# antoine311200/sow

Measured on AMD Instinct MI355X. Metric: SoWLinear fwd+bwd tokens/s, llama_60m rank=50 (56-layer SoWLinear stack), higher is better.
Workload: dtype bf16

## Files before the change

sow_amd/csrc/api.hip:

```cpp
#include "kernels.hpp"
#include <cstring>
#include <vector>
#include <cstdio>
#include <cstdlib>

namespace sow {

template <typename T, typename TO>
__global__ __launch_bounds__(256) void colsum_kernel(const T* M, int64_t ld, int64_t rows, int D, TO* out, float beta) {
  __shared__ float red[4][64];
  const int c = blockIdx.x * 64 + (threadIdx.x & 63), w = threadIdx.x >> 6;
  float s = 0.f;
  if (c < D)
    for (int64_t i = w; i < rows; i += 4) s += to_f32(M[i * ld + c]);
  red[w][threadIdx.x & 63] = s;
  __syncthreads();
  if (w == 0 && c < D) {
    float v = red[0][threadIdx.x] + red[1][threadIdx.x] + red[2][threadIdx.x] + red[3][threadIdx.x];
    if (beta != 0.f) v += beta * to_f32(out[c]);
    out[c] = from_f32<TO>(v);
  }
}
static int launch_colsum(const void* dy, int64_t T, int d_out, void* dbias, float beta, int dtype, int out_dtype,
                         hipStream_t stream) {
  const dim3 grid((d_out + 63) / 64);
  if (out_dtype != dtype && out_dtype != SOW_F32) return SOW_ERR_DTYPE;
  const bool o32 = out_dtype == SOW_F32;
  if (dtype == SOW_F32)
    hipLaunchKernelGGL((colsum_kernel<float, float>), grid, dim3(256), 0, stream, (const float*)dy, (int64_t)d_out, T, d_out, (float*)dbias, beta);
  else if (dtype == SOW_BF16 && o32)
    hipLaunchKernelGGL((colsum_kernel<bf16_t, float>), grid, dim3(256), 0, stream, (const bf16_t*)dy, (int64_t)d_out, T, d_out, (float*)dbias, beta);
  else if (dtype == SOW_BF16)
    hipLaunchKernelGGL((colsum_kernel<bf16_t, bf16_t>), grid, dim3(256), 0, stream, (const bf16_t*)dy, (int64_t)d_out, T, d_out, (bf16_t*)dbias, beta);
  else if (dtype == SOW_F16 && o32)
    hipLaunchKernelGGL((colsum_kernel<f16_t, float>), grid, dim3(256), 0, stream, (const f16_t*)dy, (int64_t)d_out, T, d_out, (float*)dbias, beta);
  else if (dtype == SOW_F16)
    hipLaunchKernelGGL((colsum_kernel<f16_t, f16_t>), grid, dim3(256), 0, stream, (const f16_t*)dy, (int64_t)d_out, T, d_out, (f16_t*)dbias, beta);
  else
    return SOW_ERR_DTYPE;
  SOW_CHECK_LAUNCH();
  return SOW_OK;
}
}

namespace sow {
static const char* const kSwitchNames[SW_COUNT] = {"FORCE_CHAIN_V1", "NO_SHORT_SPLIT", "NO_FUSED_H", "FORCE_GEMM_V1", "TN_NARROW",
                                                   "NO_GEMM3S",      "GEMM3S",         "GEMM3",      "NO_GROUPED",     "NO_PERSIST",     "NO_NT_STORE",    "NT_LOAD",        "NO_PAIR_FLUSH",  "F32_EXACT",
                                                   "NO_PARK16",      "TN_NO_NT_LOAD",  "NO_TN_ROWS",     "GEMM4",          "NO_GEMM4H",      "NO_CHAIN3F",     "NO_TN_F32Q",     "NO_SPLITK",
                                                   "NO_WIDE_CHAIN",  "NO_SHARED_X",    "NO_RAGGED",      "NO_RAGGED_GEMM", "NO_BLOCKED_QR",
                                                   "NO_SKINNY",      "NO_FUSED_ACC",   "NO_F16_TN",
                                                   "NO_H_ROWS"};
static std::atomic<int> g_switch[SW_COUNT];
static std::once_flag g_switch_once;
static void switches_from_env() {
  for (int i = 0; i < SW_COUNT; ++i) {
    char name[64];
    snprintf(name, sizeof name, "SOW_AMD_%s", kSwitchNames[i]);
    const char* v = getenv(name);
    const bool tri = i == SW_GEMM3S || i == SW_GEMM3 || i == SW_GEMM4;
    g_switch[i].store(!v ? -1 : (tri ? (v[0] != '0') : 1), std::memory_order_relaxed);
  }
}
int sw(int which) {
  std::call_once(g_switch_once, switches_from_env);
  return g_switch[which].load(std::memory_order_relaxed);
}
}

using namespace sow;

static inline size_t al256(size_t v) { return (v + 255) & ~(size_t)255; }
static inline size_t esize(int dtype) { return dtype == SOW_F32 ? 4 : 2; }
static inline bool ok_dtype(int d) { return d == SOW_F32 || d == SOW_BF16 || d == SOW_F16; }
static inline bool al4p(const void* p) { return (reinterpret_cast<uintptr_t>(p) & 3) == 0; }
static inline bool al16p(const void* p) { return (reinterpret_cast<uintptr_t>(p) & 15) == 0; }
static inline int split_dtype(int d, bool* pf) {
  d &= ~SOW_FUSE_ACC;
  *pf = (d & SOW_PARAM_F32) != 0;
  const int cd = d & ~SOW_PARAM_F32;
  if (!ok_dtype(cd) || (*pf && cd == SOW_F32)) return -1;
  return cd;
}
static inline bool flagged(int d) { return (d & SOW_PARAM_F32) != 0; }
static inline bool fuse_of(int d) { return (d & SOW_FUSE_ACC) != 0 && !flagged(d); }
static inline int nofuse(int d) { return d & ~SOW_FUSE_ACC; }

constexpr int SHORT_NTB = 128;
static inline int short_want(int ntb) { return ntb > 0 ? (256 + ntb - 1) / ntb : 1; }
static size_t short_hp_bytes(int64_t T, int d_in, int d_out, int r_live, int dtype) {
  const int ntb = ceil_div(T, 64);
  if (r_live > 64 || ntb <= 0 || ntb > SHORT_NTB) return 0;
  const int dmax = d_in > d_out ? d_in : d_out;
  int ks = short_want(ntb);
// ... 29 lines not shown
  if (nsl == 0) return SOW_OK;
  ChainParams b = p;
  const int kn = want < nsl ? want : nsl;
  b.ntb = ntb, b.st_per = 0, b.sl_per = ceil_div(nsl, kn), b.Hpartial = nullptr, b.Hload = p.Hsave, b.Hsave = nullptr;
  return f32 ? launch_chain2f(b, bwd, stream) : launch_chain2(b, bwd, dtype, stream);
}

static int gemm_auto(const void* A, int64_t lda, const void* B, int64_t ldb, bool transB, void* C, int64_t ldc,
                     const void* bias, int64_t M, int N, int K, float alpha, float beta, int dtype, hipStream_t stream,
                     void* ws = nullptr, size_t ws_bytes = 0) {
  if (dtype == SOW_F16) {
    const int g4 = sw(SW_GEMM4);
    const int64_t work = (int64_t)ceil_div(M, 256) * ceil_div(N, 256) * gemm4_splits(M, N, K, false, ws, ws_bytes);
    if (!sw_on(SW_FORCE_GEMM_V1) && (g4 > 0 || (g4 < 0 && work >= 120)) &&
        gemm4_supported(A, lda, B, ldb, transB, nullptr, 0, nullptr, 0, C, ldc, bias, M, N, K, dtype))
      return launch_gemm4(A, lda, B, ldb, transB, nullptr, 0, nullptr, 0, 0, C, ldc, bias, M, N, K, alpha, beta, stream, ws,
                          ws_bytes, dtype);
    return launch_gemm(A, lda, false, B, ldb, transB, C, ldc, bias, M, N, K, alpha, beta, dtype, stream);
  }
  if (gemm2_supported(A, lda, B, ldb, transB, nullptr, 0, nullptr, 0, C, ldc, bias, M, N, K, dtype))
    return launch_gemm2(A, lda, B, ldb, transB, nullptr, 0, nullptr, 0, 0, C, ldc, bias, M, N, K, alpha, beta, stream, ws, ws_bytes);
  return launch_gemm(A, lda, false, B, ldb, transB, C, ldc, bias, M, N, K, alpha, beta, dtype, stream);
}

extern "C" {

int sow_version(void) { return 120; }

int sow_set_switch(const char* name, int value) {
  if (!name) return SOW_ERR_NULL;
  (void)sw(0);
  for (int i = 0; i < SW_COUNT; ++i)
    if (!strcmp(name, kSwitchNames[i])) {
      g_switch[i].store(value < 0 ? -1 : (value != 0), std::memory_order_relaxed);
      return SOW_OK;
    }
  return SOW_ERR_UNSUPPORTED;
}

#ifdef SOW_STAMPS
int sow_debug_set_stamps(void* buf) {
  g_chain2_stamps = buf;
  return SOW_OK;
}
#endif

int sow_get_switch(const char* name) {
  if (!name) return SOW_ERR_NULL;
  for (int i = 0; i < SW_COUNT; ++i)
    if (!strcmp(name, kSwitchNames[i])) return sw(i);
  return SOW_ERR_UNSUPPORTED;
}

const char* sow_error_string(int code) {
  switch (code) {
    case SOW_OK: return "ok";
    case SOW_ERR_NULL: return "null pointer argument";
    case SOW_ERR_SHAPE: return "invalid shape argument";
    case SOW_ERR_DTYPE: return "unsupported dtype";
    case SOW_ERR_ALIGN: return "misaligned pointer";
    case SOW_ERR_WORKSPACE: return "workspace too small";
    case SOW_ERR_UNSUPPORTED: return "unsupported configuration";
    default: return code > 0 ? hipGetErrorString((hipError_t)code) : "unknown error";
  }
}

size_t sow_h_save_elems(int64_t T, int r_live) { return (size_t)T * (size_t)(r_live <= 64 ? 64 : r_live); }
// ... 1233 lines not shown
```

sow_amd/csrc/chain2.hip:

```cpp
#include "kernels.hpp"
#include "lds_dma.hpp"

namespace sow {

#ifdef SOW_STAMPS
#define C2_STAMP(i)                                                                                  \
  do {                                                                                               \
    if (stamps && w == 0 && lane == 0) stamps[i] = __builtin_amdgcn_s_memrealtime();                \
  } while (0)
#else
#define C2_STAMP(i) \
  do {              \
  } while (0)
#endif
#ifdef SOW_STAMPS
#define C2_TICK() __builtin_amdgcn_s_memrealtime()
#define C2_ACC(var, t0) var += __builtin_amdgcn_s_memrealtime() - (t0)
#define C2_PUT(cond, i, var)                     \
  do {                                           \
    if (stamps && (cond) && lane == 0) stamps[i] = (var); \
  } while (0)
#else
#define C2_TICK() 0ull
#define C2_ACC(var, t0) (void)(t0)
// ... 4 lines not shown

constexpr int C2_NTG = 2;
constexpr int C2_NCW = 2 * C2_NTG;
constexpr int C2_NLW = 2;
constexpr int C2_BM = 32 * C2_NTG;
#ifndef C2_DEPTH_X
#define C2_DEPTH_X 4
#define C2_NSLOT_X 6
#define C2_AHEAD_X 5
#endif
constexpr int C2_DEPTH = C2_DEPTH_X;
constexpr int C2_STAGE = 4096;
constexpr int C2_NSLOT = C2_NSLOT_X;
constexpr int C2_AHEAD = C2_AHEAD_X;
#ifdef C2_EXPERIMENT_SHALLOW_X
static_assert(C2_NSLOT == C2_AHEAD + 1 && C2_NSLOT + C2_DEPTH == 10 && C2_DEPTH >= 3 && C2_DEPTH <= 6, "80 KiB");
#else
static_assert(C2_NSLOT == C2_AHEAD + 1 && C2_NSLOT + C2_DEPTH == 10 && C2_DEPTH >= 4 && C2_DEPTH <= 6,
              "80 KiB: 8 KiB per chunk slot + 2 x 4 KiB per X slot; two 8-KiB fp32 park tiles per token group must fit its X ring");
#endif
constexpr int C2_FSLOT = 8192;
constexpr int C2_LPW = 8 / C2_NLW;
constexpr int C2_RING0 = C2_NSLOT * C2_FSLOT;
constexpr int C2_RING = C2_DEPTH * C2_STAGE;
constexpr int C2_LDS = C2_RING0 + C2_NTG * C2_RING;
constexpr int C2_THREADS = 64 * (C2_NCW + C2_NLW);
constexpr int C2_RESIDENT = 512;


template <bool TR> __device__ __forceinline__ int img_chunk(int row, int c) {
  return TR ? (c ^ (((row >> 1) & 1) << 2)) : (c ^ ((row >> 1) & 7));
}

template <typename T, bool BWD, bool P16>
__device__ __forceinline__ void chain2_block(const ChainParams& p, const int bid, char* smem, const int t, const int lane, const int w,
                                             uint64_t* stamps) {
  constexpr bool TR = !BWD;
  C2_STAMP(0);
  const int tb = p.ntb > 0 ? bid % p.ntb : bid;
  const int split = p.ntb > 0 ? bid / p.ntb : 0;
  const int64_t m0 = (int64_t)tb * C2_BM;
  const int D1 = p.D1, D2 = p.D2, rb = p.rb;
  const int nst_all = (D1 + 63) / 64, nsl_all = (D2 + 63) / 64;
  const int st0 = p.st_per > 0 ? split * p.st_per : 0;
  const int sl0 = p.sl_per > 0 ? split * p.sl_per : 0;
  const int nst = p.sl_per > 0 ? 0 : (p.st_per > 0 ? (nst_all - st0 < p.st_per ? nst_all - st0 : p.st_per) : nst_all);
  const int nsl = p.st_per > 0 ? 0 : (p.sl_per > 0 ? (nsl_all - sl0 < p.sl_per ? nsl_all - sl0 : p.sl_per) : nsl_all);
  const int total = nst + nsl;
  const T* Amat = (const T*)(BWD ? p.F2b : p.F1b);
  const T* Bmat = (const T*)(BWD ? p.F1b : p.F2b);
  const int64_t ldb = BWD ? p.ldf1b : p.ldf2b;
  const int rows_a = BWD ? D2 : D1, cols_b = BWD ? D1 : D2;
  const char* zp = zero_page_for(lane);

  if (w >= C2_NCW) {
    __builtin_amdgcn_s_setprio(3);
    const int lw = w - C2_NCW;
    const char* a_end = (const char*)(Amat + (int64_t)rows_a * rb);
    const bool own_last = rows_a > 0 && lw == ((rows_a - 1) & 63) / (8 * C2_LPW);
    uint32_t last_row_dw = 0u;
    if (own_last && lane < 32 && 2 * lane < rb) last_row_dw = *((const uint32_t*)(Amat + (int64_t)(rows_a - 1) * rb) + lane);
    asm volatile("" : "+v"(last_row_dw));
    auto chunk_is_a = [&](int c) { return BWD ? (c >= nst) : (c < nst); };
    const char* a_ptr[C2_LPW];
    const char* b_ptr[C2_LPW];
    int b_stride[C2_LPW], b_lc[C2_LPW];
#pragma unroll
    for (int ii = 0; ii < C2_LPW; ++ii) {
      const int i = C2_LPW * lw + ii;
      const int row = 8 * i + (lane >> 3), pc = lane & 7;
      const int lc = img_chunk<TR>(row, pc);
      a_ptr[ii] = (const char*)(Amat + (int64_t)row * rb) + 16 * lc;
      const bool bv = row < rb;
      b_ptr[ii] = bv ? (const char*)(Bmat + (int64_t)row * ldb + 8 * lc) : zp;
      b_stride[ii] = bv ? 128 : 0;
      b_lc[ii] = lc;
    }
    const int a_chunk_bytes = 128 * rb;
    const bool b_ragged = (cols_b & 63) != 0;
    const int nb_chunks = (cols_b + 63) / 64;
    auto issue = [&](int c) {
#ifdef C2_EXPERIMENT_NO_FACTOR_DMA
      if (c >= C2_NSLOT) return;
#endif
#ifdef C2_EXPERIMENT_HALF_FACTOR_DMA
      if (bid & 1) return;
#endif
      char* slot = smem + (c % C2_NSLOT) * C2_FSLOT;
      const int ci = c < nst ? st0 + c : sl0 + (c - nst);
      if (chunk_is_a(c)) {
#pragma unroll
        for (int ii = 0; ii < C2_LPW; ++ii) {
          const char* q = a_ptr[ii] + (int64_t)ci * a_chunk_bytes;
          dma16(q + 16 <= a_end ? (const void*)q : (const void*)zp, slot + (C2_LPW * lw + ii) * 1024);
        }
      } else {
#pragma unroll
        for (int ii = 0; ii < C2_LPW; ++ii) {
          const char* q = b_ptr[ii] + ci * b_stride[ii];
          if (b_ragged && ci == nb_chunks - 1 && ci * 64 + 8 * b_lc[ii] >= cols_b) q = zp;
          dma16((const void*)q, slot + (C2_LPW * lw + ii) * 1024);
        }
      }
    };
    const int pre = total < C2_AHEAD ? total : C2_AHEAD;
    for (int c = 0; c < pre; ++c) issue(c);
    uint64_t tw_dma = 0, tw_bar = 0;
    for (int c = 0; c < total; ++c) {
      const int newer = (total - 1 - c) < (C2_AHEAD - 1) ? (total - 1 - c) : (C2_AHEAD - 1);
      const uint64_t tk0 = C2_TICK();
      wait_groups<C2_LPW>(newer);
      C2_ACC(tw_dma, tk0);
      if (chunk_is_a(c)) {
        const int base = (c < nst ? st0 + c : sl0 + (c - nst)) * 64;
        const int lr = rows_a - 1 - base;
        if (own_last && lr >= 0 && lr < 64 && lane < 32) {
          const int cc = lane >> 2;
          *(uint32_t*)(smem + (c % C2_NSLOT) * C2_FSLOT + lr * 128 + img_chunk<TR>(lr, cc) * 16 + (lane & 3) * 4) = last_row_dw;
        }
      }
      if (c == nst) __builtin_amdgcn_s_setprio(0);
      if (c == nst) raw_barrier();
      const uint64_t tk1 = C2_TICK();
      raw_barrier();
      C2_ACC(tw_bar, tk1);
      if (c + C2_AHEAD < total) issue(c + C2_AHEAD);
    }
    C2_PUT(w == C2_NCW, 8, tw_dma);
    C2_PUT(w == C2_NCW, 9, tw_bar);
    if (nsl > 0) {
      raw_barrier();
    } else {
      raw_barrier();
    }
    raw_barrier();
    return;
  }

  if (p.pad_dst && bid * 64 < p.pad_rows) {
    const T* src = (const T*)p.pad_src;
    T* dst = (T*)p.pad_dst;
#pragma unroll
    for (int it = 0; it < 2; ++it) {
      const int idx = t + 256 * it, row = bid * 64 + (idx >> 3), c0 = (idx & 7) * 8;
      if (row < p.pad_rows) {
        u32x4 v;
        T* e = (T*)&v;
#pragma unroll
        for (int j = 0; j < 8; ++j) e[j] = (c0 + j < p.pad_r) ? src[(int64_t)row * p.pad_r + c0 + j] : (T)0.f;
        *(u32x4*)(dst + (int64_t)row * 64 + c0) = v;
      }
    }
  }
  const int tg = w & 1, hh = w >> 1;
  const int li = lane & 31, lh = lane >> 5;
  const int g = lane >> 4, jj = lane & 15, q = jj >> 2, pp = jj & 3;
  const int h2 = g >> 1;
  char* ring = smem + C2_RING0 + tg * C2_RING;
  const uint32_t ring_a = lds_addr(ring);
  const uint32_t slot_a = lds_addr(smem);
  const T* X = (const T*)p.X;
  const int64_t tok0 = m0 + 32 * tg;

  const int drow = lane >> 3, dpc = lane & 7;
  const char* xsrc[2];
  int xstride[2], xlc[2];
#pragma unroll
  for (int ii = 0; ii < 2; ++ii) {
    const int row = 8 * (2 * hh + ii) + drow;
    const int lc = dpc ^ ((row >> 1) & 7);
    const int64_t tk = tok0 + row;
    const bool v = tk < p.M;
    xsrc[ii] = v ? (const char*)(X + tk * p.ldx + lc * 8) : zp;
    xstride[ii] = v ? 128 : 0;
    xlc[ii] = lc;
  }
  const bool x_ragged = (D1 & 63) != 0;
  auto issue_x = [&](int st) {
    char* dst = ring + (st % C2_DEPTH) * C2_STAGE;
#pragma unroll
    for (int ii = 0; ii < 2; ++ii) {
      const char* qq = xsrc[ii] + (st0 + st) * xstride[ii];
      if (x_ragged && (st0 + st) * 64 + xlc[ii] * 8 >= D1) qq = zp;
      if (p.nt_load) dma16_nt((const void*)qq, dst + (2 * hh + ii) * 1024);
      else dma16((const void*)qq, dst + (2 * hh + ii) * 1024);
    }
  };

  const uint32_t xoff = (uint32_t)(li * 128);
  const int xsw = (li >> 1) & 7;
  uint32_t foff1[1], foff2;
  if constexpr (TR) {
    const int col = hh * 32 + 16 * (g & 1) + 4 * pp;
    const int r1 = 8 * h2 + q;
    foff1[0] = (uint32_t)(r1 * 128 + img_chunk<true>(r1, col >> 3) * 16 + (col & 7) * 2);
  } else {
    foff1[0] = (uint32_t)((hh * 32 + li) * 128);
  }
  if constexpr (TR) {
    const int col = hh * 32 + 16 * (g & 1) + 4 * pp;
    const int r2 = 4 * h2 + q;
    foff2 = (uint32_t)(r2 * 128 + img_chunk<true>(r2, col >> 3) * 16 + (col & 7) * 2);
  } else {
    foff2 = (uint32_t)((hh * 32 + li) * 128 + 8 * lh);
  }

  f32x16 hacc;
#pragma unroll
  for (int i = 0; i < 16; ++i) hacc[i] = 0.f;

  const int pre = nst < (C2_DEPTH - 1) ? nst : (C2_DEPTH - 1);
  for (int st = 0; st < pre; ++st) issue_x(st);

  uint64_t tw_x = 0, tw_b1 = 0, tw_b2 = 0;
#pragma unroll 1
  for (int st = 0; st < nst; ++st) {
    const int newer = (nst - 1 - st) < (C2_DEPTH - 2) ? (nst - 1 - st) : (C2_DEPTH - 2);
    const uint64_t tk0 = C2_TICK();
    wait_groups<2>(newer);
    C2_ACC(tw_x, tk0);
    const uint64_t tk1 = C2_TICK();
    raw_barrier();
    C2_ACC(tw_b1, tk1);
    if (st == 0) C2_STAMP(1);
    if (st + C2_DEPTH - 1 < nst) issue_x(st + C2_DEPTH - 1);
    const uint32_t xs = ring_a + (uint32_t)((st % C2_DEPTH) * C2_STAGE) + xoff;
    const uint32_t fs = slot_a + (uint32_t)((st % C2_NSLOT) * C2_FSLOT);
    u32x4 xf[4], ff[4];
#pragma unroll
    for (int ks = 0; ks < 4; ++ks) DS_READ_B128(xf[ks], xs + (uint32_t)(((2 * ks + lh) ^ xsw) * 16), 0);
    if constexpr (TR) {
      u32x2 bl[4], bh[4];
      const uint32_t b0 = fs + foff1[0];
      DS_READ_TR(bl[0], b0, 0);
      DS_READ_TR(bh[0], b0, 512);
      DS_READ_TR(bl[1], b0, 2048);
      DS_READ_TR(bh[1], b0, 2048 + 512);
      DS_READ_TR(bl[2], b0, 4096);
      DS_READ_TR(bh[2], b0, 4096 + 512);
      DS_READ_TR(bl[3], b0, 6144);
      DS_READ_TR(bh[3], b0, 6144 + 512);
      LGKM_WAIT0();
#pragma unroll
      for (int ks = 0; ks < 4; ++ks) ff[ks] = join2(bl[ks], bh[ks]);
    } else {
#pragma unroll
      for (int ks = 0; ks < 4; ++ks) DS_READ_B128(ff[ks], fs + foff1[0] + (uint32_t)(((2 * ks + lh) ^ xsw) * 16), 0);
      LGKM_WAIT0();
    }
#pragma unroll
    for (int ks = 0; ks < 4; ++ks) hacc = mfma32(as_v8<T>(ff[ks]), as_v8<T>(xf[ks]), hacc);
    __builtin_amdgcn_sched_barrier(0);
  }

  C2_STAMP(2);
  u32x4 hf[4];
  const int64_t tok = tok0 + li;
  if (p.Hload) {
    raw_barrier();
    const T* Hl = (const T*)p.Hload + tok * 64 + 4 * lh;
#pragma unroll
    for (int s4 = 0; s4 < 4; ++s4) {
      u32x2 lo = {0u, 0u}, hi = {0u, 0u};
      if (tok < p.M) {
        lo = *(const u32x2*)(Hl + 16 * s4);
        hi = *(const u32x2*)(Hl + 16 * s4 + 8);
      }
      if (s4 == 3 && lh == 1 && rb < 64) hi[1] &= 0xffffu;
      hf[s4] = join2(lo, hi);
    }
  } else {
    u32x4 own[2] = {{0u, 0u, 0u, 0u}, {0u, 0u, 0u, 0u}};
    if (p.Hpartial) {
      if (tok < p.M) {
        float* Hp = p.Hpartial + ((int64_t)split * p.M + tok) * 64 + hh * 32 + 4 * lh;
#pragma unroll
        for (int rq = 0; rq < 4; ++rq)
          *(f32x4*)(Hp + 8 * rq) = (f32x4){hacc[4 * rq + 0], hacc[4 * rq + 1], hacc[4 * rq + 2], hacc[4 * rq + 3]};
      }
    } else {
      float hv[16];
#pragma unroll
      for (int reg = 0; reg < 16; ++reg) {
        const int r = hh * 32 + (reg & 3) + 8 * (reg >> 2) + 4 * lh;
        hv[reg] = r < rb ? hacc[reg] * p.scale : 0.f;
      }
#pragma unroll
      for (int a = 0; a < 2; ++a)
        own[a] = (u32x4){pack16x2<T>(hv[8 * a + 0], hv[8 * a + 1]), pack16x2<T>(hv[8 * a + 2], hv[8 * a + 3]),
                         pack16x2<T>(hv[8 * a + 4], hv[8 * a + 5]), pack16x2<T>(hv[8 * a + 6], hv[8 * a + 7])};
// ... 4 lines not shown
          u32x2 v = {pack16x2<T>(hv[4 * rq + 0], hv[4 * rq + 1]), pack16x2<T>(hv[4 * rq + 2], hv[4 * rq + 3])};
          if (hh == 1 && rq == 3 && lh == 1 && rb < 64) v[1] = (v[1] & 0xffffu) | (DT<T>::one_bits << 16);
          *(u32x2*)(img + (((hh * 4 + rq) ^ ((li >> 1) & 7)) * 16)) = v;
        }
      } else if (p.Hsave && tok < p.M) {
        T* Hs = (T*)p.Hsave + tok * 64 + hh * 32 + 4 * lh;
#pragma unroll
        for (int rq = 0; rq < 4; ++rq) {
          u32x2 v = {pack16x2<T>(hv[4 * rq + 0], hv[4 * rq + 1]), pack16x2<T>(hv[4 * rq + 2], hv[4 * rq + 3])};
          if (hh == 1 && rq == 3 && lh == 1 && rb < 64) v[1] = (v[1] & 0xffffu) | (DT<T>::one_bits << 16);
          *(u32x2*)(Hs + 8 * rq) = v;
        }
      }
    }
    char* xch = ring + (nst % C2_DEPTH) * C2_STAGE;
    *(u32x4*)(xch + hh * 2048 + lane * 16) = own[0];
    *(u32x4*)(xch + hh * 2048 + 1024 + lane * 16) = own[1];
    raw_barrier();
    u32x4 oth[2];
    const uint32_t pa = ring_a + (uint32_t)((nst % C2_DEPTH) * C2_STAGE + (hh ^ 1) * 2048 + lane * 16);
    DS_READ_B128(oth[0], pa, 0);
    DS_READ_B128(oth[1], pa, 1024);
    if (p.Hsave && p.h_rows && !p.Hpartial) {
      u32x4 hr[2];
      const uint32_t ia = ring_a + (uint32_t)(((nst + 1) % C2_DEPTH) * C2_STAGE);
#pragma unroll
      for (int pass = 0; pass < 2; ++pass) {
        const int r = 16 * hh + pass * 8 + (lane >> 3);
        DS_READ_B128(hr[pass], ia + (uint32_t)(r * 128 + (((lane & 7) ^ ((r >> 1) & 7)) * 16)), 0);
      }
      LGKM_WAIT0();
#pragma unroll
      for (int pass = 0; pass < 2; ++pass) {
        const int64_t tk = tok0 + 16 * hh + pass * 8 + (lane >> 3);
        if (tk < p.M) {
          T* dst = (T*)p.Hsave + tk * 64 + (lane & 7) * 8;
          store_b128_nt(dst, hr[pass]);
        }
      }
    }
    LGKM_WAIT0();
    hf[0] = hh ? oth[0] : own[0], hf[1] = hh ? oth[1] : own[1];
    hf[2] = hh ? own[0] : oth[0], hf[3] = hh ? own[1] : oth[1];
  }
  C2_STAMP(3);
  T* Y = (T*)p.Y;
  const T* bias = (const T*)p.bias;
  const int ksteps = (rb + 15) / 16;
  auto tile_addr = [&](int buf, int row, int chunk) {
    return ring_a + (uint32_t)(buf * 8192 + row * 256 + ((chunk ^ (row & 15)) * 16));
  };
  const bool pairf = p.pair_flush != 0 && C2_RING >= 3 * 8192;
  auto flush = [&](int sl_prev) {
    const int buf = pairf ? sl_prev % 3 : (sl_prev & 1);
    u32x4 v0[2], v1[2];
#pragma unroll
    for (int pass = 0; pass < 2; ++pass) {
      const int r = 16 * hh + pass * 8 + (lane >> 3), c8 = lane & 7;
      DS_READ_B128(v0[pass], tile_addr(buf, r, 2 * c8), 0);
      DS_READ_B128(v1[pass], tile_addr(buf, r, 2 * c8 + 1), 0);
    }
    LGKM_WAIT0();
#pragma unroll
    for (int pass = 0; pass < 2; ++pass) {
      const int r = 16 * hh + pass * 8 + (lane >> 3), c8 = lane & 7;
      const int64_t tk = tok0 + r;
      const int col = (sl0 + sl_prev) * 64 + c8 * 8;
      if (tk < p.M && col < D2) {
        float v[8];
        const float* f0 = (const float*)&v0[pass];
        const float* f1 = (const float*)&v1[pass];
#pragma unroll
        for (int e = 0; e < 4; ++e) v[e] = f0[e], v[4 + e] = f1[e];
        T* dst = Y + tk * p.ldy + col;
        if (p.beta != 0.f) {
          const u32x4 old = *(const u32x4*)dst;
          const T* o = (const T*)&old;
#pragma unroll
          for (int e = 0; e < 8; ++e) v[e] += p.beta * (float)o[e];
        }
        if (bias) {
          const u32x4 bv = *(const u32x4*)(bias + col);
          const T* bb = (const T*)&bv;
#pragma unroll
          for (int e = 0; e < 8; ++e) v[e] += (float)bb[e];
        }
        const u32x4 ov = {pack16x2<T>(v[0], v[1]), pack16x2<T>(v[2], v[3]), pack16x2<T>(v[4], v[5]), pack16x2<T>(v[6], v[7])};
        if (p.nt_store) store_b128_nt(dst, ov);
        else *(u32x4*)dst = ov;
      }
    }
  };
  auto flush_pair = [&](int sl_a) {
#pragma unroll
    for (int half = 0; half < 2; ++half) {
      u32x4 v0[2], v1[2];
#pragma unroll
      for (int ps = 0; ps < 2; ++ps) {
        const int r = 16 * hh + (2 * half + ps) * 4 + (lane >> 4), c16 = lane & 15;
        const int buf = (sl_a + (c16 >> 3)) % 3, c8 = c16 & 7;
        DS_READ_B128(v0[ps], tile_addr(buf, r, 2 * c8), 0);
        DS_READ_B128(v1[ps], tile_addr(buf, r, 2 * c8 + 1), 0);
      }
      LGKM_WAIT0();
#pragma unroll
      for (int ps = 0; ps < 2; ++ps) {
        const int r = 16 * hh + (2 * half + ps) * 4 + (lane >> 4), c16 = lane & 15;
        const int64_t tk = tok0 + r;
        const int col = (sl0 + sl_a) * 64 + c16 * 8;
        if (tk < p.M && col < D2) {
          float v[8];
          const float* f0 = (const float*)&v0[ps];
          const float* f1 = (const float*)&v1[ps];
#pragma unroll
          for (int e = 0; e < 4; ++e) v[e] = f0[e], v[4 + e] = f1[e];
          T* dst = Y + tk * p.ldy + col;
          if (p.beta != 0.f) {
            const u32x4 old = *(const u32x4*)dst;
            const T* o = (const T*)&old;
#pragma unroll
            for (int e = 0; e < 8; ++e) v[e] += p.beta * (float)o[e];
          }
          if (bias) {
            const u32x4 bv = *(const u32x4*)(bias + col);
            const T* bb = (const T*)&bv;
#pragma unroll
            for (int e = 0; e < 8; ++e) v[e] += (float)bb[e];
          }
          const u32x4 ov = {pack16x2<T>(v[0], v[1]), pack16x2<T>(v[2], v[3]), pack16x2<T>(v[4], v[5]), pack16x2<T>(v[6], v[7])};
          if (p.nt_store) store_b128_nt(dst, ov);
          else *(u32x4*)dst = ov;
        }
      }
    }
  };
  constexpr bool park16 = P16;
  auto tile16_addr = [&](int buf, int row, int chunk) {
    return ring_a + (uint32_t)((C2_DEPTH - 3) * C2_STAGE + buf * 4096 + row * 128 + ((chunk ^ ((row >> 1) & 7)) * 16));
  };
  auto store16 = [&](int r, int col, u32x4 ov) {
    const int64_t tk = tok0 + r;
    if (tk < p.M && col < D2) {
      T* dst = Y + tk * p.ldy + col;
      if (p.nt_store) store_b128_nt(dst, ov);
      else *(u32x4*)dst = ov;
    }
  };
  auto flush16 = [&](int sl_prev) {
    u32x4 v[2];
#pragma unroll
    for (int pass = 0; pass < 2; ++pass) DS_READ_B128(v[pass], tile16_addr(sl_prev % 3, 16 * hh + pass * 8 + (lane >> 3), lane & 7), 0);
    LGKM_WAIT0();
#pragma unroll
    for (int pass = 0; pass < 2; ++pass) store16(16 * hh + pass * 8 + (lane >> 3), (sl0 + sl_prev) * 64 + (lane & 7) * 8, v[pass]);
  };
  auto flush_pair16 = [&](int sl_a) {
    u32x4 v[4];
#pragma unroll
    for (int ps = 0; ps < 4; ++ps) {
      const int r = 16 * hh + ps * 4 + (lane >> 4), c16 = lane & 15;
      DS_READ_B128(v[ps], tile16_addr((sl_a + (c16 >> 3)) % 3, r, c16 & 7), 0);
    }
    LGKM_WAIT0();
#pragma unroll
    for (int ps = 0; ps < 4; ++ps) store16(16 * hh + ps * 4 + (lane >> 4), (sl0 + sl_a) * 64 + (lane & 15) * 8, v[ps]);
  };
#pragma unroll 1
  for (int sl = 0; sl < nsl; ++sl) {
    const uint64_t tk2 = C2_TICK();
    raw_barrier();
    C2_ACC(tw_b2, tk2);
    const uint32_t fs = slot_a + (uint32_t)(((nst + sl) % C2_NSLOT) * C2_FSLOT) + foff2;
    u32x2 bl[4], bh[4];
    if constexpr (TR) {
      DS_READ_TR(bl[0], fs, 0);
      DS_READ_TR(bh[0], fs, 1024);
      DS_READ_TR(bl[1], fs, 2048);
      DS_READ_TR(bh[1], fs, 2048 + 1024);
      DS_READ_TR(bl[2], fs, 4096);
      DS_READ_TR(bh[2], fs, 4096 + 1024);
      DS_READ_TR(bl[3], fs, 6144);
      DS_READ_TR(bh[3], fs, 6144 + 1024);
    } else {
#pragma unroll
      for (int ks = 0; ks < 4; ++ks) {
        DS_READ_B64(bl[ks], fs + (uint32_t)(((2 * ks) ^ xsw) * 16), 0);
        DS_READ_B64(bh[ks], fs + (uint32_t)(((2 * ks + 1) ^ xsw) * 16), 0);
      }
    }
    LGKM_WAIT0();
    f32x16 yacc;
#pragma unroll
    for (int i = 0; i < 16; ++i) yacc[i] = 0.f;
#pragma unroll
    for (int ks = 0; ks < 4; ++ks)
      if (ks < ksteps) yacc = mfma32(as_v8<T>(join2(bl[ks], bh[ks])), as_v8<T>(hf[ks]), yacc);
    __builtin_amdgcn_sched_barrier(0);
    if constexpr (park16) {
      if (sl >= 2 && !(sl & 1)) flush_pair16(sl - 2);
#pragma unroll
      for (int rq = 0; rq < 4; ++rq) {
        const u32x2 v = {pack16x2<T>(yacc[4 * rq + 0], yacc[4 * rq + 1]), pack16x2<T>(yacc[4 * rq + 2], yacc[4 * rq + 3])};
        *(u32x2*)(ring + (C2_DEPTH - 3) * C2_STAGE + (sl % 3) * 4096 + li * 128 + (((hh * 4 + rq) ^ ((li >> 1) & 7)) * 16) + lh * 8) = v;
      }
    } else {
    if (pairf) {
      if (sl >= 2 && !(sl & 1)) flush_pair(sl - 2);
    } else if (sl > 0) {
      flush(sl - 1);
    }
#pragma unroll
    for (int rq = 0; rq < 4; ++rq) {
      const int chunk = hh * 8 + 2 * rq + lh;
      f32x4 v = {yacc[4 * rq + 0], yacc[4 * rq + 1], yacc[4 * rq + 2], yacc[4 * rq + 3]};
      *(f32x4*)(ring + (pairf ? sl % 3 : (sl & 1)) * 8192 + li * 256 + ((chunk ^ (li & 15)) * 16)) = v;
    }
    }
  }
  C2_STAMP(4);
  if (nsl > 0) {
    raw_barrier();
    if constexpr (park16) {
      if (nsl >= 2 && !(nsl & 1)) flush_pair16(nsl - 2);
      else flush16(nsl - 1);
    } else {
      if (pairf && nsl >= 2 && !(nsl & 1)) flush_pair(nsl - 2);
      else flush(nsl - 1);
    }
  }
  C2_STAMP(5);
  raw_barrier();
  C2_STAMP(6);
  C2_PUT(w == 0, 10, tw_x);
  C2_PUT(w == 0, 11, tw_b1);
  C2_PUT(w == 0, 12, tw_b2);
}

template <bool BWD, bool P16> __global__ __launch_bounds__(C2_THREADS, 4) void chain2_kernel(const ChainGroup grp) {
  extern __shared__ __attribute__((aligned(16))) char smem[];
  const int t = threadIdx.x;
  const int w = __builtin_amdgcn_readfirstlane(t >> 6);
  const int total = grp.start[C2_MAXG];
  for (int blk = (int)blockIdx.x; blk < total; blk += (int)gridDim.x) {
    int layer = 0;
#pragma unroll
    for (int i = 1; i < C2_MAXG; ++i)
      if (i < grp.n && blk >= grp.start[i]) layer = i;
    int tt = t;
    asm volatile("" : "+v"(tt));
    chain2_block<bf16_t, BWD, P16>(grp.p[layer], blk - grp.start[layer], smem, tt, tt & 63, w, grp.stamps ? grp.stamps + (int64_t)blk * 16 : nullptr);
  }
}
template <bool BWD, bool P16> __global__ __launch_bounds__(C2_THREADS, 4) void chain2_f16_kernel(const ChainGroup grp) {
  extern __shared__ __attribute__((aligned(16))) char smem[];
  const int t = threadIdx.x;
  const int w = __builtin_amdgcn_readfirstlane(t >> 6);
  const int total = grp.start[C2_MAXG];
  for (int blk = (int)blockIdx.x; blk < total; blk += (int)gridDim.x) {
    int layer = 0;
#pragma unroll
    for (int i = 1; i < C2_MAXG; ++i)
      if (i < grp.n && blk >= grp.start[i]) layer = i;
    int tt = t;
    asm volatile("" : "+v"(tt));
    chain2_block<f16_t, BWD, P16>(grp.p[layer], blk - grp.start[layer], smem, tt, tt & 63, w, grp.stamps ? grp.stamps + (int64_t)blk * 16 : nullptr);
  }
}

bool chain2_supported(const ChainParams& p, int dtype) {
  auto a16 = [](const void* q) { return (reinterpret_cast<uintptr_t>(q) & 15) == 0; };
  if ((dtype != SOW_BF16 && dtype != SOW_F16) || p.ra != 0 || p.rb < 4 || p.rb > 64 || (p.rb & 1)) return false;
  if (p.D1 % 8 || p.D2 % 8 || p.ldx % 8 || p.ldy % 8) return false;
  if (!a16(p.X) || !a16(p.Y) || (p.bias && !a16(p.bias)) || (p.Hsave && !a16(p.Hsave))) return false;
  if (p.M < 64) return false;
  return true;
}

template <typename T>
__global__ __launch_bounds__(256) void h_reduce_kernel(const float* __restrict__ Hp, int nsplit, T* __restrict__ Hs, int64_t M,
                                                       int rb, float scale) {
  const int64_t idx = (int64_t)blockIdx.x * 256 + threadIdx.x;
  const int64_t tok = idx >> 3;
  const int c0 = (int)(idx & 7) * 8;
  if (tok >= M) return;
  float v[8] = {0.f, 0.f, 0.f, 0.f, 0.f, 0.f, 0.f, 0.f};
  for (int s = 0; s < nsplit; ++s) {
    const f32x4 a = *(const f32x4*)(Hp + ((int64_t)s * M + tok) * 64 + c0);
    const f32x4 b = *(const f32x4*)(Hp + ((int64_t)s * M + tok) * 64 + c0 + 4);
#pragma unroll
    for (int j = 0; j < 4; ++j) v[j] += a[j], v[4 + j] += b[j];
  }
#pragma unroll
  for (int j = 0; j < 8; ++j) {
    const int c = c0 + j;
    v[j] = c < rb ? v[j] * scale : ((c == 63 && rb < 64) ? 1.0f : 0.f);
  }
  if constexpr (sizeof(T) == 2) {
    *(u32x4*)(Hs + tok * 64 + c0) = (u32x4){pack16x2<T>(v[0], v[1]), pack16x2<T>(v[2], v[3]), pack16x2<T>(v[4], v[5]), pack16x2<T>(v[6], v[7])};
// ... 29 lines not shown
  return ceil_div(p.M, C2_BM);
}

int launch_chain2_group(const ChainParams* ps, int n, bool bwd, int dtype, hipStream_t stream) {
  if (n <= 0) return SOW_OK;
  if (dtype != SOW_BF16 && dtype != SOW_F16) return SOW_ERR_DTYPE;
  if (n > C2_MAXG) return SOW_ERR_SHAPE;
  ChainGroup g{};
  g.n = n;
  int64_t total = 0;
  for (int i = 0; i < n; ++i) {
    const ChainParams& p = ps[i];
    const void* Bp = bwd ? p.F1b : p.F2b;
    const int64_t ldB = bwd ? p.ldf1b : p.ldf2b;
    const void* Ap = bwd ? p.F2b : p.F1b;
    const int64_t ldA = bwd ? p.ldf2b : p.ldf1b;
    if ((reinterpret_cast<uintptr_t>(Bp) & 15) || ldB % 8 || (reinterpret_cast<uintptr_t>(Ap) & 3) || ldA != p.rb)
      return SOW_ERR_ALIGN;
    g.p[i] = p;
    g.p[i].nt_store = sw_on(SW_NO_NT_STORE) ? 0 : 1;
    g.p[i].nt_load = sw_on(SW_NT_LOAD) ? 1 : 0;
    g.p[i].h_rows = sw_on(SW_NO_H_ROWS) ? 0 : 1;
    g.p[i].pair_flush = sw_on(SW_NO_PAIR_FLUSH) ? 0 : 1;
    g.start[i] = (int)total;
    total += chain2_grid(p);
  }
  for (int i = n; i <= C2_MAXG; ++i) g.start[i] = (int)total;
  g.stamps = (uint64_t*)g_chain2_stamps;
  if (total <= 0) return SOW_OK;
  if (total > 0x7fffffff) return SOW_ERR_SHAPE;
  const int64_t grid = (sw_on(SW_NO_PERSIST) || total < C2_RESIDENT) ? total : C2_RESIDENT;
  bool p16 = !sw_on(SW_NO_PARK16);
  for (int i = 0; i < n; ++i) p16 = p16 && g.p[i].pair_flush && g.p[i].beta == 0.f && !g.p[i].bias;
#define C2_LAUNCH(B, P)                                                                                              \
  do {                                                                                                               \
    if (dtype == SOW_F16) {                                                                                          \
      SOW_SET_MAX_LDS_ONCE(C2_LDS, (chain2_f16_kernel<B, P>));                                                       \
      hipLaunchKernelGGL((chain2_f16_kernel<B, P>), dim3((unsigned)grid), dim3(C2_THREADS), C2_LDS, stream, g);      \
    } else {                                                                                                         \
      SOW_SET_MAX_LDS_ONCE(C2_LDS, (chain2_kernel<B, P>));                                                           \
      hipLaunchKernelGGL((chain2_kernel<B, P>), dim3((unsigned)grid), dim3(C2_THREADS), C2_LDS, stream, g);          \
    }                                                                                                                \
  } while (0)
  if (bwd) {
    if (p16) C2_LAUNCH(true, true);
    else C2_LAUNCH(true, false);
  } else {
    if (p16) C2_LAUNCH(false, true);
    else C2_LAUNCH(false, false);
  }
#undef C2_LAUNCH
  SOW_CHECK_LAUNCH();
  return SOW_OK;
}

int launch_chain2(const ChainParams& p, bool bwd, int dtype, hipStream_t stream) { return launch_chain2_group(&p, 1, bwd, dtype, stream); }

}
```

sow_amd/csrc/common.hpp:

```cpp
#pragma once
#include <hip/hip_runtime.h>
#include <stdint.h>

#include <atomic>
#include <mutex>

#include "../../include/sow_amd.h"

namespace sow {

typedef __bf16 bf16_t;
typedef __attribute__((ext_vector_type(8))) __bf16 bf16x8;
typedef __attribute__((ext_vector_type(4))) __bf16 bf16x4;
typedef __attribute__((ext_vector_type(2))) __bf16 bf16x2;
typedef _Float16 f16_t;
typedef __attribute__((ext_vector_type(8))) _Float16 f16x8;
typedef __attribute__((ext_vector_type(2))) _Float16 f16x2;
typedef __attribute__((ext_vector_type(16))) float f32x16;
typedef __attribute__((ext_vector_type(4))) float f32x4;
typedef __attribute__((ext_vector_type(2))) float f32x2;
typedef __attribute__((ext_vector_type(4))) uint32_t u32x4;
typedef __attribute__((ext_vector_type(2))) uint32_t u32x2;

enum : int { SOW_F32 = 0, SOW_BF16 = 1, SOW_F16 = 2 };
// ... 96 lines not shown
  } while (0)

enum Switch : int {
  SW_FORCE_CHAIN_V1 = 0,
  SW_NO_SHORT_SPLIT,
  SW_NO_FUSED_H,
  SW_FORCE_GEMM_V1,
  SW_TN_NARROW,
  SW_NO_GEMM3S,
  SW_GEMM3S,
  SW_GEMM3,
  SW_NO_GROUPED,
  SW_NO_PERSIST,
  SW_NO_NT_STORE,
  SW_NT_LOAD,
  SW_NO_PAIR_FLUSH,
  SW_F32_EXACT,
  SW_NO_PARK16,
  SW_TN_NO_NT_LOAD,
  SW_NO_TN_ROWS,
  SW_GEMM4,
  SW_NO_GEMM4H,
  SW_NO_CHAIN3F,
  SW_NO_TN_F32Q,
  SW_NO_SPLITK,
  SW_NO_WIDE_CHAIN,
  SW_NO_SHARED_X,
  SW_NO_RAGGED,
  SW_NO_RAGGED_GEMM,
  SW_NO_BLOCKED_QR,
  SW_NO_SKINNY,
  SW_NO_FUSED_ACC,
  SW_NO_F16_TN,
  SW_NO_H_ROWS,
  SW_COUNT
};
int sw(int which);
inline bool sw_on(int which) { return sw(which) > 0; }

#ifdef SOW_GEMM_NO_NT
#define SOW_GEMM_NT(M) false
#else
#define SOW_GEMM_NT(M) ((M) >= 8192)
#endif

#define SOW_CHECK_LAUNCH()                     \
  do {                                         \
    hipError_t e__ = hipGetLastError();        \
    if (e__ != hipSuccess) return (int)e__;    \
  } while (0)

}
```

sow_amd/csrc/kernels.hpp:

```cpp
#pragma once
#include "common.hpp"

namespace sow {
struct ChainParams {
  const void* X;
  void* Y;
  const void *F1a, *F1b, *F2a, *F2b;
  void* Hsave;
  const void* bias;
  int64_t M, ldx, ldy, ldf1a, ldf1b, ldf2a, ldf2b;
  int D1, D2, ra, rb;
  float scale, beta;
  int fast_factors;
  const void* pad_src;
  void* pad_dst;
  int pad_rows, pad_r;
  int ntb, st_per, sl_per;
  float* Hpartial;
  const void* Hload;
  int nt_store;
  int nt_load;
  int h_rows;
  int pair_flush;
  void* planes;
  size_t planes_bytes;
};
int launch_chain(ChainParams p, int dtype, bool bwd, hipStream_t stream);
constexpr int C2_MAXG = 4;
struct ChainGroup {
  ChainParams p[C2_MAXG];
  int start[C2_MAXG + 1];
  int n;
  uint64_t* stamps;
};
extern void* g_chain2_stamps;
bool chain2_supported(const ChainParams& p, int dtype);
int launch_chain2(const ChainParams& p, bool bwd, int dtype, hipStream_t stream);
int launch_chain2_group(const ChainParams* ps, int n, bool bwd, int dtype, hipStream_t stream);
bool chain2_shared_supported(const ChainParams* ps, int n, bool bwd, int dtype);
int launch_chain2_shared(const ChainParams* ps, int n, bool bwd, int dtype, hipStream_t stream);
int launch_h_reduce(const float* Hpartial, int nsplit, void* Hsave, int64_t M, int rb, float scale, int dtype,
                    hipStream_t stream);
bool chain2f_supported(const ChainParams& p, int dtype);
int launch_chain2f(const ChainParams& p, bool bwd, hipStream_t stream);
size_t chain3f_plane_bytes(int d_in, int d_out);
bool chain3f_supported(const ChainParams& p, int dtype);
int launch_chain3f(const ChainParams& p, bool bwd, hipStream_t stream);
struct TnJob {
  const void* M;
  const void* S;
  float* partial;
  int64_t ldm;
  int D;
  int ones_col;
  int ncg;
  int vec;
// ... 238 lines not shown
```

Before: 8.964 million.

## Align half-offset row loads and stores in chain2 via interleaved token parity

Adds a row-align mode to the chain2 kernel. It triggers when a row stride is 32 mod 64 elements and the feature dimension has a half-chunk remainder. Token groups then take interleaved rows by parity, and odd rows are shifted by 32 elements, so their X loads and Y stores start on 128-byte boundaries. To cover the shifted data, factor chunks are read across the previous and current LDS slots, and the prefetch depth drops by one. The aim is to remove misaligned global accesses, at the cost of reduced DMA lookahead and more complex indexing that could carry correctness risk.

New measurement: 9.068 million (median of 6 runs). 1.2% higher.

```diff
diff --git a/sow_amd/csrc/api.hip b/sow_amd/csrc/api.hip
--- a/sow_amd/csrc/api.hip
+++ b/sow_amd/csrc/api.hip
@@ -49,7 +49,7 @@
                                                    "NO_PARK16",      "TN_NO_NT_LOAD",  "NO_TN_ROWS",     "GEMM4",          "NO_GEMM4H",      "NO_CHAIN3F",     "NO_TN_F32Q",     "NO_SPLITK",
                                                    "NO_WIDE_CHAIN",  "NO_SHARED_X",    "NO_RAGGED",      "NO_RAGGED_GEMM", "NO_BLOCKED_QR",
                                                    "NO_SKINNY",      "NO_FUSED_ACC",   "NO_F16_TN",
-                                                   "NO_H_ROWS"};
+                                                   "NO_ROW_ALIGN",   "NO_H_ROWS"};
 static std::atomic<int> g_switch[SW_COUNT];
 static std::once_flag g_switch_once;
 static void switches_from_env() {
@@ -58,7 +58,8 @@
     snprintf(name, sizeof name, "SOW_AMD_%s", kSwitchNames[i]);
     const char* v = getenv(name);
     const bool tri = i == SW_GEMM3S || i == SW_GEMM3 || i == SW_GEMM4;
-    g_switch[i].store(!v ? -1 : (tri ? (v[0] != '0') : 1), std::memory_order_relaxed);
+    const int on = i == SW_NO_ROW_ALIGN && v && v[0] >= '1' && v[0] <= '3' ? v[0] - '0' : 1;
+    g_switch[i].store(!v ? -1 : (tri ? (v[0] != '0') : on), std::memory_order_relaxed);
   }
 }
 int sw(int which) {
@@ -154,7 +155,7 @@
   (void)sw(0);
   for (int i = 0; i < SW_COUNT; ++i)
     if (!strcmp(name, kSwitchNames[i])) {
-      g_switch[i].store(value < 0 ? -1 : (value != 0), std::memory_order_relaxed);
+      g_switch[i].store(value < 0 ? -1 : (i == SW_NO_ROW_ALIGN && value <= 3 ? value : (value != 0)), std::memory_order_relaxed);
       return SOW_OK;
     }
   return SOW_ERR_UNSUPPORTED;
diff --git a/sow_amd/csrc/chain2.hip b/sow_amd/csrc/chain2.hip
--- a/sow_amd/csrc/chain2.hip
+++ b/sow_amd/csrc/chain2.hip
@@ -60,7 +60,7 @@
   return TR ? (c ^ (((row >> 1) & 1) << 2)) : (c ^ ((row >> 1) & 7));
 }
 
-template <typename T, bool BWD, bool P16>
+template <typename T, bool BWD, bool P16, bool AL>
 __device__ __forceinline__ void chain2_block(const ChainParams& p, const int bid, char* smem, const int t, const int lane, const int w,
                                              uint64_t* stamps) {
   constexpr bool TR = !BWD;
@@ -80,6 +80,7 @@
   const int64_t ldb = BWD ? p.ldf1b : p.ldf2b;
   const int rows_a = BWD ? D2 : D1, cols_b = BWD ? D1 : D2;
   const char* zp = zero_page_for(lane);
+  const int ral = AL ? p.row_align : 0;
 
   if (w >= C2_NCW) {
     __builtin_amdgcn_s_setprio(3);
@@ -131,11 +132,12 @@
         }
       }
     };
-    const int pre = total < C2_AHEAD ? total : C2_AHEAD;
+    const int ahead = ral ? C2_AHEAD - 1 : C2_AHEAD;
+    const int pre = total < ahead ? total : ahead;
     for (int c = 0; c < pre; ++c) issue(c);
     uint64_t tw_dma = 0, tw_bar = 0;
     for (int c = 0; c < total; ++c) {
-      const int newer = (total - 1 - c) < (C2_AHEAD - 1) ? (total - 1 - c) : (C2_AHEAD - 1);
+      const int newer = (total - 1 - c) < (ahead - 1) ? (total - 1 - c) : (ahead - 1);
       const uint64_t tk0 = C2_TICK();
       wait_groups<C2_LPW>(newer);
       C2_ACC(tw_dma, tk0);
@@ -152,7 +154,7 @@
       const uint64_t tk1 = C2_TICK();
       raw_barrier();
       C2_ACC(tw_bar, tk1);
-      if (c + C2_AHEAD < total) issue(c + C2_AHEAD);
+      if (c + ahead < total) issue(c + ahead);
     }
     C2_PUT(w == C2_NCW, 8, tw_dma);
     C2_PUT(w == C2_NCW, 9, tw_bar);
@@ -188,7 +190,10 @@
   const uint32_t ring_a = lds_addr(ring);
   const uint32_t slot_a = lds_addr(smem);
   const T* X = (const T*)p.X;
-  const int64_t tok0 = m0 + 32 * tg;
+  const bool par = ral != 0;
+  const bool ord = par && tg == 1 && (ral & 1), owr = P16 && par && tg == 1 && (ral & 2);
+  auto trow = [&](int r) -> int64_t { return m0 + (par ? 2 * r + tg : 32 * tg + r); };
+  const int xsh = ord ? 32 : 0, ysh = owr ? 32 : 0;
 
   const int drow = lane >> 3, dpc = lane & 7;
   const char* xsrc[2];
@@ -197,9 +202,9 @@
   for (int ii = 0; ii < 2; ++ii) {
     const int row = 8 * (2 * hh + ii) + drow;
     const int lc = dpc ^ ((row >> 1) & 7);
-    const int64_t tk = tok0 + row;
+    const int64_t tk = trow(row);
     const bool v = tk < p.M;
-    xsrc[ii] = v ? (const char*)(X + tk * p.ldx + lc * 8) : zp;
+    xsrc[ii] = v ? (const char*)(X + tk * p.ldx + lc * 8 - xsh) : zp;
     xstride[ii] = v ? 128 : 0;
     xlc[ii] = lc;
   }
@@ -209,7 +214,12 @@
 #pragma unroll
     for (int ii = 0; ii < 2; ++ii) {
       const char* qq = xsrc[ii] + (st0 + st) * xstride[ii];
-      if (x_ragged && (st0 + st) * 64 + xlc[ii] * 8 >= D1) qq = zp;
+      if constexpr (AL) {
+        const int col = (st0 + st) * 64 + xlc[ii] * 8 - xsh;
+        if ((x_ragged || xsh) && (col < 0 || col >= D1)) qq = zp;
+      } else {
+        if (x_ragged && (st0 + st) * 64 + xlc[ii] * 8 >= D1) qq = zp;
+      }
       if (p.nt_load) dma16_nt((const void*)qq, dst + (2 * hh + ii) * 1024);
       else dma16((const void*)qq, dst + (2 * hh + ii) * 1024);
     }
@@ -225,12 +235,13 @@
   } else {
     foff1[0] = (uint32_t)((hh * 32 + li) * 128);
   }
+  const int ct = owr ? hh ^ 1 : hh;
   if constexpr (TR) {
-    const int col = hh * 32 + 16 * (g & 1) + 4 * pp;
+    const int col = ct * 32 + 16 * (g & 1) + 4 * pp;
     const int r2 = 4 * h2 + q;
     foff2 = (uint32_t)(r2 * 128 + img_chunk<true>(r2, col >> 3) * 16 + (col & 7) * 2);
   } else {
-    foff2 = (uint32_t)((hh * 32 + li) * 128 + 8 * lh);
+    foff2 = (uint32_t)((ct * 32 + li) * 128 + 8 * lh);
   }
 
   f32x16 hacc;
@@ -254,11 +265,24 @@
     if (st + C2_DEPTH - 1 < nst) issue_x(st + C2_DEPTH - 1);
     const uint32_t xs = ring_a + (uint32_t)((st % C2_DEPTH) * C2_STAGE) + xoff;
     const uint32_t fs = slot_a + (uint32_t)((st % C2_NSLOT) * C2_FSLOT);
+    const uint32_t fsp = AL && ord && st > 0 ? slot_a + (uint32_t)(((st - 1) % C2_NSLOT) * C2_FSLOT) : fs;
     u32x4 xf[4], ff[4];
 #pragma unroll
     for (int ks = 0; ks < 4; ++ks) DS_READ_B128(xf[ks], xs + (uint32_t)(((2 * ks + lh) ^ xsw) * 16), 0);
     if constexpr (TR) {
       u32x2 bl[4], bh[4];
+      if constexpr (AL) {
+        const uint32_t b0 = fsp + foff1[0] + (ord ? 4096u : 0u);
+        const uint32_t b1 = fs + foff1[0] + (ord ? 0u : 4096u);
+        DS_READ_TR(bl[0], b0, 0);
+        DS_READ_TR(bh[0], b0, 512);
+        DS_READ_TR(bl[1], b0, 2048);
+        DS_READ_TR(bh[1], b0, 2048 + 512);
+        DS_READ_TR(bl[2], b1, 0);
+        DS_READ_TR(bh[2], b1, 512);
+        DS_READ_TR(bl[3], b1, 2048);
+        DS_READ_TR(bh[3], b1, 2048 + 512);
+      } else {
       const uint32_t b0 = fs + foff1[0];
       DS_READ_TR(bl[0], b0, 0);
       DS_READ_TR(bh[0], b0, 512);
@@ -268,22 +292,39 @@
       DS_READ_TR(bh[2], b0, 4096 + 512);
       DS_READ_TR(bl[3], b0, 6144);
       DS_READ_TR(bh[3], b0, 6144 + 512);
+      }
       LGKM_WAIT0();
 #pragma unroll
       for (int ks = 0; ks < 4; ++ks) ff[ks] = join2(bl[ks], bh[ks]);
     } else {
 #pragma unroll
-      for (int ks = 0; ks < 4; ++ks) DS_READ_B128(ff[ks], fs + foff1[0] + (uint32_t)(((2 * ks + lh) ^ xsw) * 16), 0);
+      for (int ks = 0; ks < 4; ++ks) {
+        if constexpr (AL) {
+          const int kk = (ks + (ord ? 2 : 0)) & 3;
+          DS_READ_B128(ff[ks], (ks < 2 ? fsp : fs) + foff1[0] + (uint32_t)(((2 * kk + lh) ^ xsw) * 16), 0);
+        } else {
+          DS_READ_B128(ff[ks], fs + foff1[0] + (uint32_t)(((2 * ks + lh) ^ xsw) * 16), 0);
+        }
+      }
       LGKM_WAIT0();
     }
+    if constexpr (AL) {
+      if (!(ord && st == 0)) {
+        hacc = mfma32(as_v8<T>(ff[0]), as_v8<T>(xf[0]), hacc);
+        hacc = mfma32(as_v8<T>(ff[1]), as_v8<T>(xf[1]), hacc);
+      }
+      hacc = mfma32(as_v8<T>(ff[2]), as_v8<T>(xf[2]), hacc);
+      hacc = mfma32(as_v8<T>(ff[3]), as_v8<T>(xf[3]), hacc);
+    } else {
 #pragma unroll
     for (int ks = 0; ks < 4; ++ks) hacc = mfma32(as_v8<T>(ff[ks]), as_v8<T>(xf[ks]), hacc);
+    }
     __builtin_amdgcn_sched_barrier(0);
   }
 
   C2_STAMP(2);
   u32x4 hf[4];
-  const int64_t tok = tok0 + li;
+  const int64_t tok = trow(li);
   if (p.Hload) {
     raw_barrier();
     const T* Hl = (const T*)p.Hload + tok * 64 + 4 * lh;
@@ -354,7 +395,7 @@
       LGKM_WAIT0();
 #pragma unroll
       for (int pass = 0; pass < 2; ++pass) {
-        const int64_t tk = tok0 + 16 * hh + pass * 8 + (lane >> 3);
+        const int64_t tk = trow(16 * hh + pass * 8 + (lane >> 3));
         if (tk < p.M) {
           T* dst = (T*)p.Hsave + tk * 64 + (lane & 7) * 8;
           store_b128_nt(dst, hr[pass]);
@@ -386,7 +427,7 @@
 #pragma unroll
     for (int pass = 0; pass < 2; ++pass) {
       const int r = 16 * hh + pass * 8 + (lane >> 3), c8 = lane & 7;
-      const int64_t tk = tok0 + r;
+      const int64_t tk = trow(r);
       const int col = (sl0 + sl_prev) * 64 + c8 * 8;
       if (tk < p.M && col < D2) {
         float v[8];
@@ -428,7 +469,7 @@
 #pragma unroll
       for (int ps = 0; ps < 2; ++ps) {
         const int r = 16 * hh + (2 * half + ps) * 4 + (lane >> 4), c16 = lane & 15;
-        const int64_t tk = tok0 + r;
+        const int64_t tk = trow(r);
         const int col = (sl0 + sl_a) * 64 + c16 * 8;
         if (tk < p.M && col < D2) {
           float v[8];
@@ -461,8 +502,8 @@
     return ring_a + (uint32_t)((C2_DEPTH - 3) * C2_STAGE + buf * 4096 + row * 128 + ((chunk ^ ((row >> 1) & 7)) * 16));
   };
   auto store16 = [&](int r, int col, u32x4 ov) {
-    const int64_t tk = tok0 + r;
-    if (tk < p.M && col < D2) {
+    const int64_t tk = trow(r);
+    if (tk < p.M && col < D2 && (!AL || col >= 0)) {
       T* dst = Y + tk * p.ldy + col;
       if (p.nt_store) store_b128_nt(dst, ov);
       else *(u32x4*)dst = ov;
@@ -474,7 +515,7 @@
     for (int pass = 0; pass < 2; ++pass) DS_READ_B128(v[pass], tile16_addr(sl_prev % 3, 16 * hh + pass * 8 + (lane >> 3), lane & 7), 0);
     LGKM_WAIT0();
 #pragma unroll
-    for (int pass = 0; pass < 2; ++pass) store16(16 * hh + pass * 8 + (lane >> 3), (sl0 + sl_prev) * 64 + (lane & 7) * 8, v[pass]);
+    for (int pass = 0; pass < 2; ++pass) store16(16 * hh + pass * 8 + (lane >> 3), (sl0 + sl_prev) * 64 + (lane & 7) * 8 - ysh, v[pass]);
   };
   auto flush_pair16 = [&](int sl_a) {
     u32x4 v[4];
@@ -485,14 +526,15 @@
     }
     LGKM_WAIT0();
 #pragma unroll
-    for (int ps = 0; ps < 4; ++ps) store16(16 * hh + ps * 4 + (lane >> 4), (sl0 + sl_a) * 64 + (lane & 15) * 8, v[ps]);
+    for (int ps = 0; ps < 4; ++ps) store16(16 * hh + ps * 4 + (lane >> 4), (sl0 + sl_a) * 64 + (lane & 15) * 8 - ysh, v[ps]);
   };
 #pragma unroll 1
   for (int sl = 0; sl < nsl; ++sl) {
     const uint64_t tk2 = C2_TICK();
     raw_barrier();
     C2_ACC(tw_b2, tk2);
-    const uint32_t fs = slot_a + (uint32_t)(((nst + sl) % C2_NSLOT) * C2_FSLOT) + foff2;
+    const int fc = nst + sl - ((AL && owr && hh == 0 && sl > 0) ? 1 : 0);
+    const uint32_t fs = slot_a + (uint32_t)((fc % C2_NSLOT) * C2_FSLOT) + foff2;
     u32x2 bl[4], bh[4];
     if constexpr (TR) {
       DS_READ_TR(bl[0], fs, 0);
@@ -558,7 +600,7 @@
   C2_PUT(w == 0, 12, tw_b2);
 }
 
-template <bool BWD, bool P16> __global__ __launch_bounds__(C2_THREADS, 4) void chain2_kernel(const ChainGroup grp) {
+template <bool BWD, bool P16, bool AL> __global__ __launch_bounds__(C2_THREADS, 4) void chain2_kernel(const ChainGroup grp) {
   extern __shared__ __attribute__((aligned(16))) char smem[];
   const int t = threadIdx.x;
   const int w = __builtin_amdgcn_readfirstlane(t >> 6);
@@ -570,10 +612,10 @@
       if (i < grp.n && blk >= grp.start[i]) layer = i;
     int tt = t;
     asm volatile("" : "+v"(tt));
-    chain2_block<bf16_t, BWD, P16>(grp.p[layer], blk - grp.start[layer], smem, tt, tt & 63, w, grp.stamps ? grp.stamps + (int64_t)blk * 16 : nullptr);
-  }
-}
-template <bool BWD, bool P16> __global__ __launch_bounds__(C2_THREADS, 4) void chain2_f16_kernel(const ChainGroup grp) {
+    chain2_block<bf16_t, BWD, P16, AL>(grp.p[layer], blk - grp.start[layer], smem, tt, tt & 63, w, grp.stamps ? grp.stamps + (int64_t)blk * 16 : nullptr);
+  }
+}
+template <bool BWD, bool P16, bool AL> __global__ __launch_bounds__(C2_THREADS, 4) void chain2_f16_kernel(const ChainGroup grp) {
   extern __shared__ __attribute__((aligned(16))) char smem[];
   const int t = threadIdx.x;
   const int w = __builtin_amdgcn_readfirstlane(t >> 6);
@@ -585,7 +627,7 @@
       if (i < grp.n && blk >= grp.start[i]) layer = i;
     int tt = t;
     asm volatile("" : "+v"(tt));
-    chain2_block<f16_t, BWD, P16>(grp.p[layer], blk - grp.start[layer], smem, tt, tt & 63, w, grp.stamps ? grp.stamps + (int64_t)blk * 16 : nullptr);
+    chain2_block<f16_t, BWD, P16, AL>(grp.p[layer], blk - grp.start[layer], smem, tt, tt & 63, w, grp.stamps ? grp.stamps + (int64_t)blk * 16 : nullptr);
   }
 }
 
@@ -681,15 +723,33 @@
   const int64_t grid = (sw_on(SW_NO_PERSIST) || total < C2_RESIDENT) ? total : C2_RESIDENT;
   bool p16 = !sw_on(SW_NO_PARK16);
   for (int i = 0; i < n; ++i) p16 = p16 && g.p[i].pair_flush && g.p[i].beta == 0.f && !g.p[i].bias;
-#define C2_LAUNCH(B, P)                                                                                              \
+  const int no_al = sw(SW_NO_ROW_ALIGN);
+  bool al = false;
+  for (int i = 0; i < n; ++i) {
+    ChainParams& q = g.p[i];
+    auto half_off = [](const void* base, int64_t ld, int D) {
+      return ld % 64 == 32 && D % 64 > 0 && D % 64 <= 32 && (reinterpret_cast<uintptr_t>(base) & 127) == 0;
+    };
+    q.row_align = 0;
+    if (q.ntb > 0) continue;
+    if (no_al != 1 && no_al != 2 && half_off(q.X, q.ldx, q.D1)) q.row_align |= 1;
+    if (no_al != 1 && no_al != 3 && p16 && half_off(q.Y, q.ldy, q.D2)) q.row_align |= 2;
+    al = al || q.row_align != 0;
+  }
+#define C2_LAUNCH_AL(B, P, A)                                                                                        \
   do {                                                                                                               \
     if (dtype == SOW_F16) {                                                                                          \
-      SOW_SET_MAX_LDS_ONCE(C2_LDS, (chain2_f16_kernel<B, P>));                                                       \
-      hipLaunchKernelGGL((chain2_f16_kernel<B, P>), dim3((unsigned)grid), dim3(C2_THREADS), C2_LDS, stream, g);      \
+      SOW_SET_MAX_LDS_ONCE(C2_LDS, (chain2_f16_kernel<B, P, A>));                                                    \
+      hipLaunchKernelGGL((chain2_f16_kernel<B, P, A>), dim3((unsigned)grid), dim3(C2_THREADS), C2_LDS, stream, g);   \
     } else {                                                                                                         \
-      SOW_SET_MAX_LDS_ONCE(C2_LDS, (chain2_kernel<B, P>));                                                           \
-      hipLaunchKernelGGL((chain2_kernel<B, P>), dim3((unsigned)grid), dim3(C2_THREADS), C2_LDS, stream, g);          \
+      SOW_SET_MAX_LDS_ONCE(C2_LDS, (chain2_kernel<B, P, A>));                                                        \
+      hipLaunchKernelGGL((chain2_kernel<B, P, A>), dim3((unsigned)grid), dim3(C2_THREADS), C2_LDS, stream, g);       \
     }                                                                                                                \
+  } while (0)
+#define C2_LAUNCH(B, P)                \
+  do {                                 \
+    if (al) C2_LAUNCH_AL(B, P, true);  \
+    else C2_LAUNCH_AL(B, P, false);    \
   } while (0)
   if (bwd) {
     if (p16) C2_LAUNCH(true, true);
@@ -699,6 +759,7 @@
     else C2_LAUNCH(false, false);
   }
 #undef C2_LAUNCH
+#undef C2_LAUNCH_AL
   SOW_CHECK_LAUNCH();
   return SOW_OK;
 }
diff --git a/sow_amd/csrc/common.hpp b/sow_amd/csrc/common.hpp
--- a/sow_amd/csrc/common.hpp
+++ b/sow_amd/csrc/common.hpp
@@ -152,6 +152,7 @@
   SW_NO_SKINNY,
   SW_NO_FUSED_ACC,
   SW_NO_F16_TN,
+  SW_NO_ROW_ALIGN,
   SW_NO_H_ROWS,
   SW_COUNT
 };
diff --git a/sow_amd/csrc/kernels.hpp b/sow_amd/csrc/kernels.hpp
--- a/sow_amd/csrc/kernels.hpp
+++ b/sow_amd/csrc/kernels.hpp
@@ -22,6 +22,7 @@
   int nt_load;
   int h_rows;
   int pair_flush;
+  int row_align;
   void* planes;
   size_t planes_bytes;
 };
```
